# lianqi1008/Control-GIC

Measured on AMD Instinct MI355X. Metric: encode+decode MPixels/s at fixed granularity ratio; bpp match vs reference, higher is better.
Workload: dtype f32; 1 GPU; batch 64 of 256x256 per GPU per step, codebook 1024x4, ratio (0.1,0.8,0.1), hot path only (entropy maps + router + VQ + Huffman/mask coder, encode+decode); conv encoder/decoder out of scope, latent synthetic; inputs=8 distinct resident batches in rotation (416 MiB > 256 MiB Infinity Cache)

## Files before the change

control-gic_amd/csrc/cgic_decode.hip:

```cpp
#include "cgic_coder_dev.h"

#include <atomic>

namespace cgic {

constexpr int kWinBytes = 8192;
constexpr int kWinWords = kWinBytes / 4 + 4;

struct WaveDecoder {
    const TableDev &t;
    const uint32_t *lut;
    uint32_t *win;
    const uint8_t *in;
    int nbytes;
    int wb;

    __device__ __forceinline__ void fill(int first_byte)
    {
        const int lane = lane_id();
        wb = first_byte & ~3;
        const uintptr_t g = reinterpret_cast<uintptr_t>(in) + (uintptr_t)wb;
        const uint32_t *ga = reinterpret_cast<const uint32_t *>(g & ~(uintptr_t)3);
        wsh = (int)(g & 3);
        const int limit = (nbytes - wb + wsh + 3) / 4 + 2;
// ... 592 lines not shown
            decode_segmented<false>(a.tab, lut, win + wave * kSegWinWords, seg, in, nb, s_pad, 0, wave < nw ? nw : 0, wave, cap, put,
                                    &s_count, ft);
        else
            decode_segmented<true>(a.tab, lut, win + wave * kSegWinWords, seg, in, nb, s_pad, 0, wave < nw ? nw : 0, wave, cap, put,
                                   &s_count, ft);
        __syncthreads();
        if (tid == 0) *dc = s_count > cap ? -3 : s_count;
        return;
    }
    PartSync ps{a.bf + (b * 3 + s) * kDecPartsMax * kWave, a.tick + (b * 3 + s) * kTicketStride, s_entry};
    int nbits = s_pad == 0 ? 0 : (nb - 1) * 8 - s_pad;
    nbits = nbits < 0 ? 0 : nbits;
    const int nchunks = (nbits + kWave - 1) / kWave, per_part = (nchunks + nparts - 1) / nparts;
    if (per_part <= kFastChunks) {
        decode_segmented<true>(a.tab, lut, win + wave * kSegWinWords, seg, in, nb, s_pad, 0, kDecWaves, wave, cap, put, &s_count, ft,
                               part, nparts, 0, 0, nullptr, &ps);
    } else {
        decode_segmented<false>(a.tab, lut, win + wave * kSegWinWords, seg, in, nb, s_pad, 0, kDecWaves, wave, 0,
                                [](int, int) {}, &s_count, (FastTables *)nullptr, part, nparts, 0, 0, s_fn);
        __syncthreads();
        if (wave == 0) part_exchange(part, nparts, s_fn[tid], ps);
        if (tid == 0) s_count = 0;
        __syncthreads();
        decode_segmented<true>(a.tab, lut, win + wave * kSegWinWords, seg, in, nb, s_pad, 0, kDecWaves, wave, cap, put, &s_count, ft,
                               part, nparts, s_entry[0], s_entry[1]);
    }
    __syncthreads();
    if (tid == 0 && part == nparts - 1) *dc = s_count > cap ? -3 : s_count;
}

__global__ __launch_bounds__(kDecThreads) void decode_split_kernel(DecodeArgs a)
{
    decode_split_body(a, own_blk());
}

__global__ __launch_bounds__(kDecThreads) void decode_split_grouped_kernel(Grouped<DecodeArgs> g)
{
    Blk blk;
    decode_split_body(g.a[group_locate(g, &blk)], blk);
}

struct MergeArgs {
    const uint8_t *in;
    int64_t slot;
    const int32_t *nbytes;
    int64_t h, w;
    int mode;
    const uint16_t *dsym;
    const int32_t *dcount;
    int64_t *ind_out;
    int32_t *mc_out, *mm_out, *mf_out;
    const float *codebook;
    int K;
    float *zq;
    const float *codebook2;
    float *zq2;
    int32_t *status;
    int stage_sym, stage_cb;
    int64_t band_syms;
};

__device__ __forceinline__ void wait_decoded(unsigned int *done, unsigned int need, unsigned int total)
{
    if (threadIdx.x == 0) {
        while (__hip_atomic_load(done, __ATOMIC_RELAXED, __HIP_MEMORY_SCOPE_AGENT) < need) __builtin_amdgcn_s_sleep(8);
        const unsigned int old = __hip_atomic_fetch_add(done, 1u, __ATOMIC_RELAXED, __HIP_MEMORY_SCOPE_AGENT);
        if (old + 1u == total) __hip_atomic_store(done, 0u, __ATOMIC_RELAXED, __HIP_MEMORY_SCOPE_AGENT);
        __builtin_amdgcn_fence(__ATOMIC_ACQUIRE, "agent");
    }
    __syncthreads();
}

typedef unsigned int cgic_u32x4 __attribute__((ext_vector_type(4)));
typedef unsigned int cgic_u32x2 __attribute__((ext_vector_type(2)));
__device__ __forceinline__ void nt_store16(void *p, const void *v)
{
    __builtin_nontemporal_store(*reinterpret_cast<const cgic_u32x4 *>(v), reinterpret_cast<cgic_u32x4 *>(p));
}
__device__ __forceinline__ void nt_store8(void *p, const void *v)
{
    __builtin_nontemporal_store(*reinterpret_cast<const cgic_u32x2 *>(v), reinterpret_cast<cgic_u32x2 *>(p));
}

template <int NT, bool WAIT = false>
__device__ __forceinline__ void merge_body(const MergeArgs &a, const Blk blk, unsigned int *done = nullptr, unsigned int need = 0,
                                           unsigned int total = 0)
{
    extern __shared__ __attribute__((aligned(16))) uint32_t sm[];
    __shared__ uint32_t scan_smem[NT / kWave + 1];
    __shared__ int s_status;
    __shared__ int s_hdr[8];
    const int tid = threadIdx.x;
    const int band = blk.x;
    const int64_t b = blk.y;
    const int64_t h = a.h, w = a.w, h2 = h >> 1, w2 = w >> 1, h4 = h >> 2, w4 = w >> 2;
    const int64_t n_c = h4 * w4, n_m = h2 * w2, n_f = h * w;
    const int64_t wc = (n_c + 31) >> 5, wm = (n_m + 31) >> 5;
    const int64_t nsym = n_c + n_m + n_f;
    float4 *cbk = reinterpret_cast<float4 *>(sm);
    uint16_t *lsym = reinterpret_cast<uint16_t *>(cbk + (a.stage_cb ? a.K : 0));
    uint32_t *rawc = reinterpret_cast<uint32_t *>(lsym) + (a.stage_sym ? (nsym + 1) / 2 : 0);
    uint32_t *rawm = rawc + wc + 2;
    uint32_t *mcb = rawm + wm + 2;
    uint32_t *mmb = mcb + wc;
    uint32_t *pcb = mmb + wm;
    uint32_t *pmb = pcb + wc;
    const int mode = a.mode;
    const int64_t nbands = blk.nx;
    const int64_t rows_per = ((h4 + nbands - 1) / nbands) * 4;
    const int64_t r0 = band * rows_per, r1 = r0 + rows_per < h ? r0 + rows_per : h;
    if (r0 >= h) return;
    CGIC_STAMP(10);
    const bool send_mc = mode == 0 || mode == 2 || mode == 3;
    const bool send_mm = mode == 0 || mode == 1;
    const uint8_t *in_mc = a.in + (b * CGIC_NUM_STREAMS + 3) * a.slot;
    const uint8_t *in_mm = a.in + (b * CGIC_NUM_STREAMS + 4) * a.slot;

    if (tid == 0) s_status = 0;
    if (tid < 2) s_hdr[tid] = a.nbytes[b * CGIC_NUM_STREAMS + 3 + tid];
    else if (!WAIT && tid < 5) s_hdr[tid] = a.dcount[b * 3 + (tid - 2)];
    if (send_mc) for (int64_t i = tid; i < wc + 2; i += NT) rawc[i] = reinterpret_cast<const uint32_t *>(in_mc)[i];
    if (send_mm) for (int64_t i = tid; i < wm + 2; i += NT) rawm[i] = reinterpret_cast<const uint32_t *>(in_mm)[i];
    const uint16_t *gsym = a.dsym + b * nsym;
    if (!WAIT && a.stage_sym) {
        const uint32_t *g32 = reinterpret_cast<const uint32_t *>(gsym);
        uint32_t *l32 = reinterpret_cast<uint32_t *>(lsym);
        for (int64_t i = tid; i < (nsym + 1) / 2; i += NT) l32[i] = g32[i];
    }
    if (a.stage_cb && a.zq)
        for (int i = tid; i < a.K; i += NT) cbk[i] = reinterpret_cast<const float4 *>(a.codebook)[i];
    __syncthreads();
    CGIC_STAMP(11);

    if (tid == 0) {
        if (send_mc && (s_hdr[0] != 2 + (n_c >> 3) || (int)(rawc[0] & 0xFF) != 8 - (int)(n_c & 7))) s_status = CGIC_ERR_INVALID;
        if (send_mm && (s_hdr[1] != 2 + (n_m >> 3) || (int)(rawm[0] & 0xFF) != 8 - (int)(n_m & 7))) s_status = CGIC_ERR_INVALID;
    }
    __syncthreads();
    if (s_status) {
        if (WAIT) wait_decoded(done, need, total);
        if (tid == 0 && a.status) atomicMin(&a.status[b], s_status);
        return;
    }
    auto stream_word = [](const uint32_t *raw, int64_t wi, int64_t nbits) -> uint32_t {
        const uint64_t two = (uint64_t)raw[wi] | ((uint64_t)raw[wi + 1] << 32);
        const uint32_t pay = (uint32_t)(two >> 8);
        uint32_t v = __builtin_bswap32(__brev(pay));
        const int64_t rem = nbits - wi * 32;
        if (rem < 32) v &= rem <= 0 ? 0u : ((1u << rem) - 1u);
        return v;
    };
    uint32_t cnt_c, cnt_m;
    __shared__ uint32_t s_cnt[2];
    const bool derived_mm = mode == 3 || mode == 5;
    if (wc <= kWave && wm <= kWave && !derived_mm) {
        const int lane = lane_id(), wave = tid >> 6;
        if (wave < 2) {
            const bool co = wave == 0;
            const int64_t nw_ = co ? wc : wm, nb_ = co ? n_c : n_m;
            uint32_t v = 0;
            if (lane < nw_) {
                if (co ? send_mc : send_mm) v = stream_word(co ? rawc : rawm, lane, nb_);
                else if (co && mode == 4) {
                    v = 0xFFFFFFFFu;
                    const int64_t rem = nb_ - (int64_t)lane * 32;
                    if (rem < 32) v &= (1u << rem) - 1u;
                }
            }
            const uint32_t c = (uint32_t)__popc(v);
            const uint32_t inc = wave_inclusive_scan(c);
            if (lane < nw_) {
                (co ? mcb : mmb)[lane] = v;
                (co ? pcb : pmb)[lane] = inc - c;
            }
            if (lane == kWave - 1) s_cnt[wave] = inc;
        }
        __syncthreads();
        cnt_c = s_cnt[0];
        cnt_m = s_cnt[1];
    } else {
        for (int64_t i = tid; i < wc; i += NT) {
            uint32_t v = 0;
            if (send_mc) v = stream_word(rawc, i, n_c);
            else if (mode == 4) {
                v = 0xFFFFFFFFu;
                const int64_t rem = n_c - i * 32;
                if (rem < 32) v &= (1u << rem) - 1u;
            }
            mcb[i] = v;
        }
        __syncthreads();
        for (int64_t i = tid; i < wm; i += NT) {
            uint32_t v = 0;
            if (send_mm) v = stream_word(rawm, i, n_m);
            else if (mode == 3 || mode == 5) {
                for (int k = 0; k < 32; ++k) {
                    const int64_t j = i * 32 + k;
                    if (j >= n_m) break;
                    bool bit = true;
                    if (mode == 3) {
                        const int64_t y = j / w2, x = j - y * w2, c = (y >> 1) * w4 + (x >> 1);
                        bit = !((mcb[c >> 5] >> (c & 31)) & 1u);
                    }
                    v |= (uint32_t)bit << k;
                }
            }
            mmb[i] = v;
        }
        __syncthreads();
        if (wc <= NT && wm <= NT) {
            __shared__ unsigned long long scan64[NT / kWave + 1];
            const unsigned long long c = ((unsigned long long)(tid < wc ? __popc(mcb[tid]) : 0) << 32) | (unsigned long long)(tid < wm ? __popc(mmb[tid]) : 0);
            unsigned long long tot;
            const unsigned long long ex = block_exclusive_scan(c, scan64, &tot);
            if (tid < wc) pcb[tid] = (uint32_t)(ex >> 32);
            if (tid < wm) pmb[tid] = (uint32_t)ex;
            cnt_c = (uint32_t)(tot >> 32);
            cnt_m = (uint32_t)tot;
            __syncthreads();
        } else {
        uint32_t carry = 0, total;
        for (int64_t base = 0; base < wc; base += NT) {
            const int64_t i = base + tid;
            const uint32_t c = i < wc ? (uint32_t)__popc(mcb[i]) : 0u;
            const uint32_t ex = block_exclusive_scan(c, scan_smem, &total);
            if (i < wc) pcb[i] = carry + ex;
            carry += total;
        }
        cnt_c = carry;
        carry = 0;
        for (int64_t base = 0; base < wm; base += NT) {
            const int64_t i = base + tid;
            const uint32_t c = i < wm ? (uint32_t)__popc(mmb[i]) : 0u;
            const uint32_t ex = block_exclusive_scan(c, scan_smem, &total);
            if (i < wm) pmb[i] = carry + ex;
            carry += total;
        }
        cnt_m = carry;
        __syncthreads();
        }
    }
    CGIC_STAMP(12);

    auto fine_flag = [&](int64_t y, int64_t x, bool *pbc, bool *pbm) -> bool {
        const int64_t j2 = (y >> 1) * w2 + (x >> 1), j4 = (y >> 2) * w4 + (x >> 2);
        const bool bc = (mcb[j4 >> 5] >> (j4 & 31)) & 1u;
        const bool bm = (mmb[j2 >> 5] >> (j2 & 31)) & 1u;
        *pbc = bc; *pbm = bm;
        switch (mode) {
        case 0: return (1 - (int)bm - (int)bc) == 1;
        case 1: return !bm;
        case 2: return !bc;
        case 6: return true;
        default: return false;
        }
    };
    uint32_t fbase = 0;
    {
        uint32_t mine = 0;
        const int wvm = tid >> 6, lnm = tid & 63;
        for (int y2 = wvm; y2 < (int)(r0 >> 1); y2 += NT / 64)
            for (int x2 = lnm; x2 < (int)w2; x2 += 64) {
                bool bc, bm;
                mine += fine_flag(2 * y2, 2 * x2, &bc, &bm) ? 4u : 0u;
            }
        (void)block_exclusive_scan(mine, scan_smem, &fbase);
    }
    CGIC_STAMP(13);
    if (WAIT) {
        wait_decoded(done, need, total);
        if (tid >= 2 && tid < 5) s_hdr[tid] = a.dcount[b * 3 + (tid - 2)];
        if (a.stage_sym) {
            const uint32_t *g32 = reinterpret_cast<const uint32_t *>(gsym);
            uint32_t *l32 = reinterpret_cast<uint32_t *>(lsym);
            for (int64_t i = tid; i < (nsym + 1) / 2; i += NT) l32[i] = g32[i];
        }
        __syncthreads();
    }

    const uint16_t *ds_c = a.stage_sym ? lsym : gsym, *ds_m = ds_c + n_c, *ds_f = ds_m + n_m;
    const int64_t dc_c = s_hdr[2], dc_m = s_hdr[3], dc_f = s_hdr[4];
    uint16_t *bsym = reinterpret_cast<uint16_t *>(pmb + wm);
    int64_t off_c = 0, off_m = 0, off_f = 0;
    if (!a.stage_sym && a.band_syms > 0) {
        auto rank_of = [&](const uint32_t *bits, const uint32_t *pre, int64_t j, int64_t nbits, uint32_t total) -> int64_t {
            if (j >= nbits) return (int64_t)total;
            return (int64_t)pre[j >> 5] + __popc(bits[j >> 5] & ((1u << (j & 31)) - 1u));
        };
        const int64_t c0 = rank_of(mcb, pcb, (r0 >> 2) * w4, n_c, cnt_c), c1 = rank_of(mcb, pcb, (r1 >> 2) * w4, n_c, cnt_c);
        const int64_t m0 = rank_of(mmb, pmb, (r0 >> 1) * w2, n_m, cnt_m), m1 = rank_of(mmb, pmb, (r1 >> 1) * w2, n_m, cnt_m);
        const int64_t f0 = fbase, f1 = f0 + (r1 - r0) * w;
        const int64_t nc = c1 - c0, nm = m1 - m0, nf = (f1 < n_f ? f1 : n_f) - f0;
        if (nc >= 0 && nm >= 0 && nf >= 0 && nc + nm + nf + 3 <= a.band_syms) {
            for (int64_t i = tid; i < nc; i += NT) bsym[i] = ds_c[c0 + i];
            for (int64_t i = tid; i < nm; i += NT) bsym[nc + i] = ds_m[m0 + i];
            for (int64_t i = tid; i < nf; i += NT) bsym[nc + nm + i] = ds_f[f0 + i];
            __syncthreads();
            off_c = c0; off_m = m0 - nc; off_f = f0 - nc - nm;
            ds_c = bsym; ds_m = bsym; ds_f = bsym;
        }
    }
    const bool has_c = mode == 0 || mode == 2 || mode == 3 || mode == 4;
    const bool has_m = mode == 0 || mode == 1 || mode == 3 || mode == 5;
    const bool has_f = mode == 0 || mode == 1 || mode == 2 || mode == 6;
    int st = 0;
    if (dc_c == -3 || dc_m == -3 || dc_f == -3) st = CGIC_ERR_INVALID;
    if (has_c && dc_c >= 0 && dc_c != cnt_c) st = CGIC_ERR_INVALID;
    if (has_m && dc_m >= 0 && dc_m != cnt_m) st = CGIC_ERR_INVALID;
    const bool use_c = has_c && dc_c >= 0, use_m = has_m && dc_m >= 0, use_f = has_f && dc_f >= 0;

    int64_t *ind_out = a.ind_out ? a.ind_out + b * n_f : nullptr;
    float *zq = a.zq ? a.zq + b * 4 * n_f : nullptr;
    float *zq2 = a.zq2 ? a.zq2 + b * 4 * n_f : nullptr;
    uint32_t fcarry = fbase;
    int bad_index = 0;
    const int w4i = (int)w4;
    for (int64_t qbase = r0 * w4; qbase < r1 * w4; qbase += NT) {
        const int64_t q = qbase + tid;
        const bool live = q < r1 * w4;
        int64_t v[4] = {0, 0, 0, 0};
        bool bfa = false, bfb = false;
        int y = 0, xq = 0;
        if (live) {
            y = (int)q / w4i; xq = (int)q - y * w4i;
            const int64_t j4 = (int64_t)(y >> 2) * w4 + xq, j2 = (int64_t)(y >> 1) * w2 + 2 * xq;
            bool bc, bma, bmb, dummy;
            bfa = fine_flag(y, 4 * xq, &bc, &bma);
            bfb = fine_flag(y, 4 * xq + 2, &dummy, &bmb);
            int64_t vc = 0, va = 0, vb = 0;
            if (bc && use_c) vc = ds_c[(int64_t)pcb[j4 >> 5] + __popc(mcb[j4 >> 5] & ((1u << (j4 & 31)) - 1u)) - off_c];
            if (use_m) {
                const uint32_t word = mmb[j2 >> 5], below = word & ((1u << (j2 & 31)) - 1u);
                const int64_t rk = (int64_t)pmb[j2 >> 5] + __popc(below) - off_m;
                if (bma) va = ds_m[rk];
                if (bmb) vb = ds_m[rk + (bma ? 1 : 0)];
            }
            v[0] = v[1] = vc + va;
            v[2] = v[3] = vc + vb;
            const int64_t i = (int64_t)y * w + 4 * xq;
            if (a.mc_out && (y & 3) == 0) a.mc_out[b * n_c + j4] = bc;
            if (a.mm_out && (y & 1) == 0) { const int2 t2 = make_int2(bma, bmb); nt_store8(a.mm_out + b * n_m + j2, &t2); }
            if (a.mf_out) { const int4 t4 = make_int4(bfa, bfa, bfb, bfb); nt_store16(a.mf_out + b * n_f + i, &t4); }
        }
        uint32_t ftotal;
        uint32_t frank = block_exclusive_scan((bfa ? 2u : 0u) + (bfb ? 2u : 0u), scan_smem, &ftotal) + fcarry;
        if (live) {
            if (bfa) {
                if (use_f) {
                    if ((int64_t)frank < dc_f) v[0] += ds_f[(int64_t)frank - off_f];
                    if ((int64_t)frank + 1 < dc_f) v[1] += ds_f[(int64_t)frank + 1 - off_f];
                }
                frank += 2;
            }
            if (bfb && use_f) {
                if ((int64_t)frank < dc_f) v[2] += ds_f[(int64_t)frank - off_f];
                if ((int64_t)frank + 1 < dc_f) v[3] += ds_f[(int64_t)frank + 1 - off_f];
            }
            const int64_t i = (int64_t)y * w + 4 * xq;
            if (ind_out) {
                nt_store16(ind_out + i, &v[0]);
                nt_store16(ind_out + i + 2, &v[2]);
            }
            if (zq || zq2) {
#pragma unroll
                for (int k = 0; k < 4; ++k)
                    if (v[k] < 0 || v[k] >= a.K) { bad_index = 1; v[k] = 0; }
            }
            if (zq) {
                float4 e[4];
#pragma unroll
                for (int k = 0; k < 4; ++k) e[k] = a.stage_cb ? cbk[v[k]] : reinterpret_cast<const float4 *>(a.codebook)[v[k]];
                const float4 o0 = make_float4(e[0].x, e[1].x, e[2].x, e[3].x), o1 = make_float4(e[0].y, e[1].y, e[2].y, e[3].y);
                const float4 o2 = make_float4(e[0].z, e[1].z, e[2].z, e[3].z), o3 = make_float4(e[0].w, e[1].w, e[2].w, e[3].w);
                nt_store16(zq + i, &o0);
                nt_store16(zq + n_f + i, &o1);
                nt_store16(zq + 2 * n_f + i, &o2);
                nt_store16(zq + 3 * n_f + i, &o3);
            }
            if (zq2) {
                float4 e[4];
#pragma unroll
                for (int k = 0; k < 4; ++k) e[k] = reinterpret_cast<const float4 *>(a.codebook2)[v[k]];
                *reinterpret_cast<float4 *>(zq2 + i) = make_float4(e[0].x, e[1].x, e[2].x, e[3].x);
                *reinterpret_cast<float4 *>(zq2 + n_f + i) = make_float4(e[0].y, e[1].y, e[2].y, e[3].y);
                *reinterpret_cast<float4 *>(zq2 + 2 * n_f + i) = make_float4(e[0].z, e[1].z, e[2].z, e[3].z);
                *reinterpret_cast<float4 *>(zq2 + 3 * n_f + i) = make_float4(e[0].w, e[1].w, e[2].w, e[3].w);
            }
        }
        fcarry += ftotal;
    }
    CGIC_STAMP(14);
    if (r1 == h && has_f && (dc_f >= 0 ? dc_f != (int64_t)fcarry : fcarry != 0)) st = CGIC_ERR_INVALID;
    if (bad_index) s_status = CGIC_ERR_INVALID;
    __syncthreads();
    if (tid == 0 && a.status && (st || s_status)) atomicMin(&a.status[b], st ? st : s_status);
}

template <int NT>
__global__ __launch_bounds__(NT) void merge_kernel(MergeArgs a)
{
    merge_body<NT>(a, own_blk());
}

__global__ __launch_bounds__(kMergeThreads) void merge_grouped_kernel(Grouped<MergeArgs> g)
{
    Blk blk;
    merge_body<kMergeThreads>(g.a[group_locate(g, &blk)], blk);
}

struct DecodeMergeArgs {
    DecodeArgs c;
    MergeArgs m;
    unsigned int *done;
    unsigned int ndec, nbands, active_bands, B;
};
__device__ __forceinline__ void decode_merge_body(const DecodeMergeArgs &p, const unsigned int id)
{
    const unsigned int ndec_all = p.ndec * p.B;
    if (id < ndec_all) {
        const unsigned int b = id / p.ndec;
        decode_split_body(p.c, Blk{id - b * p.ndec, b, 0u, p.ndec, p.B});
        __syncthreads();
        if (threadIdx.x == 0) {
            __builtin_amdgcn_fence(__ATOMIC_RELEASE, "agent");
            __hip_atomic_fetch_add(p.done + (size_t)b * kTicketStride, 1u, __ATOMIC_RELAXED, __HIP_MEMORY_SCOPE_AGENT);
        }
        return;
    }
    const unsigned int r = id - ndec_all, b = r / p.nbands;
    merge_body<kDecThreads, true>(p.m, Blk{r - b * p.nbands, b, 0u, p.nbands, p.B}, p.done + (size_t)b * kTicketStride, p.ndec,
                                  p.ndec + p.active_bands);
}
__global__ __launch_bounds__(kDecThreads) void decode_merge_kernel(DecodeMergeArgs p)
{
    decode_merge_body(p, blockIdx.x);
}
__global__ __launch_bounds__(kDecThreads) void decode_merge_grouped_kernel(Grouped<DecodeMergeArgs> g)
{
    Blk blk;
    const DecodeMergeArgs &p = g.a[group_locate(g, &blk)];
    decode_merge_body(p, blk.x);
}

__global__ void gather_kernel(const int64_t *__restrict__ ind, int64_t B, int64_t hw,
                              const float *__restrict__ cb, int K, float *__restrict__ out,
                              int32_t *__restrict__ status)
{
    const int64_t n = B * hw;
    for (int64_t i = (int64_t)blockIdx.x * blockDim.x + threadIdx.x; i < n; i += (int64_t)gridDim.x * blockDim.x) {
        int64_t v = ind[i];
        const int64_t b = i / hw, p = i - b * hw;
        if (v < 0 || v >= K) { if (status) status[b] = CGIC_ERR_INVALID; v = 0; }
        const float4 e = reinterpret_cast<const float4 *>(cb)[v];
        float *o = out + b * 4 * hw + p;
        o[0] = e.x; o[hw] = e.y; o[2 * hw] = e.z; o[3 * hw] = e.w;
    }
}

}

using namespace cgic;

static size_t decoder_lds_bytes(bool fast_tables)
{
    const size_t seg = sizeof(uint32_t) * (kDecLutMax + kDecWaves * kSegWinWords) + sizeof(SegShared) + sizeof(int32_t) * 2 * kLdsTrieNodes
                       + (fast_tables ? sizeof(FastTables) : 0);
    const size_t one_wave = sizeof(uint32_t) * (kDecLutMax + kWinWords);
    return seg > one_wave ? seg : one_wave;
}

extern "C" int cgic_decode_stream(const cgic_table *t, const uint8_t *in, int64_t nbytes, int64_t *syms,
                                  int64_t cap, int64_t *count, cgic_stream_t stream)
{
    CGIC_NOT_IN_GROUP("cgic_decode_stream");
    CGIC_REQUIRE(t && count && (in || nbytes == 0) && (syms || cap == 0), CGIC_ERR_INVALID, "decode_stream: NULL argument");
    CGIC_REQUIRE(nbytes >= 0 && cap >= 0 && nbytes < ((int64_t)1 << 28), CGIC_ERR_INVALID, "decode_stream: size out of range");
    DecodeOneArgs a;
    int rc = table_device_view(t, &a.tab);
    if (rc) return rc;
    a.in = in; a.nbytes = nbytes; a.syms = syms; a.cap = cap; a.count = count;
    const size_t lds = decoder_lds_bytes(false);
    rc = ensure_dynamic_lds((const void *)decode_stream_kernel, lds);
    if (rc) return rc;
    hipLaunchKernelGGL(decode_stream_kernel, dim3(1), dim3(kDecThreads), lds, (hipStream_t)stream, a);
    return launch_check("decode_stream_kernel");
}

static std::atomic<int> g_decode_mode{CGIC_DECODE_AUTO};
static std::atomic<unsigned int *> g_decode_stats{nullptr};
extern "C" int cgic_decode_stats(unsigned int *device_counters)
{
    CGIC_REQUIRE(((uintptr_t)device_counters & 3u) == 0, CGIC_ERR_INVALID, "decode_stats: the counters must be 4-byte aligned");
    g_decode_stats.store(device_counters, std::memory_order_relaxed);
    return CGIC_OK;
}
extern "C" int cgic_set_decode_mode(int mode)
{
    CGIC_REQUIRE(mode == CGIC_DECODE_AUTO || mode == CGIC_DECODE_LATENCY || mode == CGIC_DECODE_THROUGHPUT, CGIC_ERR_INVALID,
                 "set_decode_mode: mode %d", mode);
    return g_decode_mode.exchange(mode);
}

extern "C" size_t cgic_decompress_workspace_bytes(int64_t B, int64_t h, int64_t w)
{
    if (B <= 0 || h <= 0 || w <= 0) return 0;
    const size_t per = (size_t)((h / 4) * (w / 4) + (h / 2) * (w / 2) + h * w);
    return align16((size_t)B * per * sizeof(uint16_t)) + align16((size_t)B * 3 * sizeof(int32_t))
           + align16((size_t)B * 3 * kDecPartsMax * kWave * sizeof(uint32_t));
}

extern "C" int cgic_decompress_streams(const cgic_table *t, const uint8_t *in, int64_t slot, const int32_t *nbytes,
                                       int64_t B, int64_t h, int64_t w, int mode, int64_t *ind_out,
                                       int32_t *mask_c_out, int32_t *mask_m_out, int32_t *mask_f_out,
                                       const float *codebook, int K, int e_dim, float *z_q, const float *codebook2,
                                       float *z_q2, int32_t *status,
                                       void *workspace, int decoder, cgic_stream_t stream)
{
    int rc = check_grid(B, h, w, mode);
    if (rc) return rc;
    CGIC_REQUIRE(t && in && nbytes && workspace, CGIC_ERR_INVALID, "decompress_streams: NULL argument");
    CGIC_REQUIRE(decoder == CGIC_DECODE_AUTO || decoder == CGIC_DECODE_LATENCY || decoder == CGIC_DECODE_THROUGHPUT, CGIC_ERR_INVALID,
                 "decompress_streams: decoder %d", decoder);
    const int dec_mode = decoder != CGIC_DECODE_AUTO ? decoder : g_decode_mode.load();
    CGIC_REQUIRE(slot % 16 == 0 && slot >= 16 && slot < ((int64_t)1 << 28), CGIC_ERR_INVALID,
                 "decompress_streams: slot must be a multiple of 16 below 2^28");
    CGIC_REQUIRE(!z_q || (codebook && e_dim == 4 && K > 0), CGIC_ERR_UNSUPPORTED,
                 "decompress_streams: fused gather needs a [K,4] codebook");
    CGIC_REQUIRE(!z_q2 || (codebook2 && e_dim == 4 && K > 0), CGIC_ERR_UNSUPPORTED,
                 "decompress_streams: the second gather needs a [K,4] table");
    CGIC_REQUIRE(cgic_table_num_symbols(t) <= 65536, CGIC_ERR_UNSUPPORTED, "table too large");
    CGIC_REQUIRE(((reinterpret_cast<uintptr_t>(ind_out) | reinterpret_cast<uintptr_t>(z_q) | reinterpret_cast<uintptr_t>(z_q2) |
                   reinterpret_cast<uintptr_t>(mask_f_out)) & 15) == 0 && (reinterpret_cast<uintptr_t>(mask_m_out) & 7) == 0,
                 CGIC_ERR_INVALID, "decompress_streams: outputs must be 16-byte aligned");
    if (B == 0) return CGIC_OK;
    hipStream_t s = (hipStream_t)stream;
    DecodeArgs d;
    rc = table_device_view(t, &d.tab);
    if (rc) return rc;

    DecodeShape shape;
    shape.B = B; shape.h = h; shape.w = w; shape.slot = slot; shape.K = K; shape.has_zq = z_q != nullptr;
    shape.max_len = d.tab.max_len; shape.lut_bits = d.tab.lut_bits; shape.dec_mode = dec_mode;
    rc = device_cu_count(&shape.cus);
    if (rc) return rc;
// ... 116 lines not shown
```

control-gic_amd/csrc/cgic_decode_ss.hip:

```cpp
#include "cgic_coder_dev.h"

namespace cgic {

constexpr int kSsEnd = 0xFF;

struct SsLayout {
    int nbits[3];
    int c[4];
    int off[3];
};
__device__ __forceinline__ int sel3(int s, int v0, int v1, int v2) { return s == 0 ? v0 : (s == 1 ? v1 : v2); }

__device__ __forceinline__ uint32_t ss_bits(uint32_t d0, uint32_t d1, uint32_t d2, int pos)
{
    const uint32_t hi = pos < 32 ? d0 : d1, lo = pos < 32 ? d1 : d2;
    const uint32_t r = __builtin_amdgcn_alignbit(hi, lo, 32u - ((uint32_t)pos & 31u));
    return (pos & 31) ? r : hi;
}

template <bool WRITE, typename Put>
__device__ __forceinline__ int ss_walk(const TableDev &t, const uint32_t *lut, const uint8_t *stage, const SsLayout &L, int g,
                                       int entry, int *count, Put put)
{
    const int s = (g >= L.c[1]) + (g >= L.c[2]);
    const int ch = g - sel3(s, L.c[0], L.c[1], L.c[2]);
    const int rem = sel3(s, L.nbits[0], L.nbits[1], L.nbits[2]) - 64 * ch;
    *count = 0;
    if (entry == kSsEnd) return kSsEnd;
    const uint32_t *q = reinterpret_cast<const uint32_t *>(stage + sel3(s, L.off[0], L.off[1], L.off[2]) + 8 * ch);
    const uint32_t r0 = __builtin_bswap32(q[0]), r1 = __builtin_bswap32(q[1]), r2 = __builtin_bswap32(q[2]),
                   r3 = __builtin_bswap32(q[3]), r4 = __builtin_bswap32(q[4]);
    const uint32_t d0 = __builtin_amdgcn_alignbit(r0, r1, 24), d1 = __builtin_amdgcn_alignbit(r1, r2, 24),
                   d2 = __builtin_amdgcn_alignbit(r2, r3, 24), d3 = __builtin_amdgcn_alignbit(r3, r4, 24);
    const int LB = t.lut_bits;
    int pos = entry, n = 0;
    if (t.max_len <= LB) {
        const uint32_t a0 = pos < 32 ? d0 : d1, a1 = pos < 32 ? d1 : d2, a2 = pos < 32 ? d2 : d3, a3 = pos < 32 ? d3 : 0u;
        const uint32_t sft = 32u - ((uint32_t)pos & 31u);
        const bool al = ((uint32_t)pos & 31u) == 0u;
        uint32_t w0 = al ? a0 : __builtin_amdgcn_alignbit(a0, a1, sft), w1 = al ? a1 : __builtin_amdgcn_alignbit(a1, a2, sft),
                 w2 = al ? a2 : __builtin_amdgcn_alignbit(a2, a3, sft);
        const int remc = rem < 128 ? rem : 128, lim = rem < 64 ? rem : 64;
        const uint32_t ish = 30u - (uint32_t)LB;
        const uint32_t imask = ((1u << LB) - 1u) << 2;
        const char *lutb = reinterpret_cast<const char *>(lut);
        auto step = [&]() {
            const bool go = pos < lim;
            const uint32_t e = *reinterpret_cast<const uint32_t *>(lutb + ((w0 >> ish) & imask));
            const int len = (int)(e & 0xFF);
            const int np = pos + len;
            const bool ok = go && np <= remc;
            if (WRITE) { if (ok) put(s, n, (int)(e >> 8)); }
            const uint32_t r = 32u - (uint32_t)len;
            w0 = __builtin_amdgcn_alignbit(w0, w1, r);
            w1 = __builtin_amdgcn_alignbit(w1, w2, r);
            w2 <<= (len & 31);
            pos = go ? np : pos;
            n += ok ? 1 : 0;
        };
        while (__builtin_amdgcn_ballot_w64(pos < lim) != 0) {
            step();
            step();
        }
        *count = n;
        return (pos < 64 || pos > remc) ? kSsEnd : pos - 64;
    }
    while (pos < 64) {
        if (pos >= rem) { *count = n; return kSsEnd; }
        const uint32_t bits = ss_bits(d0, d1, d2, pos);
        const uint32_t e = lut[bits >> (32 - LB)];
        int len = (int)(e & 0xFF), sym = (int)(e >> 8);
        if (len == 0) {
            if (sym == 0xFFFFFF) { *count = n; return kSsEnd; }
            const unsigned long long w0 = ((unsigned long long)d0 << 32) | d1, w1 = ((unsigned long long)d2 << 32) | d3;
            const unsigned long long win = pos ? (w0 << pos) | (w1 >> (64 - pos)) : w0;
            int node = sym, k = LB;
            sym = -1;
            while (pos + k < rem && k < 64) {
                const int c = t.child[2 * node + (int)((win >> (63 - k)) & 1ull)];
                ++k;
                if (c == INT32_MIN) break;
                if (c < 0) { sym = ~c; break; }
                node = c;
            }
            if (sym < 0) { *count = n; return kSsEnd; }
            len = k;
        }
        if (pos + len > rem) { *count = n; return kSsEnd; }
        if (WRITE) put(s, n, sym);
        pos += len;
        ++n;
    }
    *count = n;
    return pos - 64;
}


constexpr int kSsMaxSweeps = 32;
constexpr int kMeEntries = 15;
constexpr uint32_t kMeEnd = 15;

struct MeFn { uint32_t r[4]; };

__device__ __forceinline__ MeFn me_identity() { return MeFn{{0x03020100u, 0x07060504u, 0x0B0A0908u, 0x0F0E0D0Cu}}; }
__device__ __forceinline__ MeFn me_const0() { return MeFn{{0u, 0u, 0u, 0u}}; }
__device__ __forceinline__ MeFn me_compose(const MeFn &prev, const MeFn &cur)
{
    MeFn o;
#pragma unroll
    for (int k = 0; k < 4; ++k) {
        const uint32_t sel = prev.r[k];
        const uint32_t s7 = sel & 0x07070707u;
        const uint32_t lo = __builtin_amdgcn_perm(cur.r[1], cur.r[0], s7);
        const uint32_t hi = __builtin_amdgcn_perm(cur.r[3], cur.r[2], s7);
        const uint32_t m = ((sel >> 3) & 0x01010101u) * 0xFFu;
        o.r[k] = (hi & m) | (lo & ~m);
    }
    return o;
}
__device__ __forceinline__ uint32_t me_apply(const MeFn &f, uint32_t e)
{
    const uint32_t w = e < 8 ? (e < 4 ? f.r[0] : f.r[1]) : (e < 12 ? f.r[2] : f.r[3]);
    return (w >> (8 * (e & 3))) & 0xFFu;
}
__device__ __forceinline__ MeFn me_shfl_up(const MeFn &f, int d)
{
    MeFn o;
#pragma unroll
    for (int k = 0; k < 4; ++k) o.r[k] = (uint32_t)__shfl_up((int)f.r[k], d, kWave);
    return o;
}
__device__ __forceinline__ MeFn me_wave_scan(MeFn f)
{
    const int lane = lane_id();
#pragma unroll
    for (int d = 1; d < kWave; d <<= 1) {
        const MeFn p = me_shfl_up(f, d);
        const MeFn c = me_compose(p, f);
        if (lane >= d) f = c;
    }
    return f;
}

__device__ __forceinline__ MeFn me_walk_all(const TableDev &t, const uint32_t *lut, const uint8_t *stage, const SsLayout &L, int g,
                                            unsigned long long *cnt_lo, unsigned long long *cnt_hi)
{
    const int s = (g >= L.c[1]) + (g >= L.c[2]);
    const int ch = g - sel3(s, L.c[0], L.c[1], L.c[2]);
    const int rem = sel3(s, L.nbits[0], L.nbits[1], L.nbits[2]) - 64 * ch;
    const uint32_t *q = reinterpret_cast<const uint32_t *>(stage + sel3(s, L.off[0], L.off[1], L.off[2]) + 8 * ch);
    const uint32_t r0 = __builtin_bswap32(q[0]), r1 = __builtin_bswap32(q[1]), r2 = __builtin_bswap32(q[2]), r3 = __builtin_bswap32(q[3]);
    const uint32_t d0 = __builtin_amdgcn_alignbit(r0, r1, 24), d1 = __builtin_amdgcn_alignbit(r1, r2, 24), d2 = __builtin_amdgcn_alignbit(r2, r3, 24);
    const int LB = t.lut_bits;
    const int remc = rem < 128 ? rem : 128, lim = rem < 64 ? rem : 64;
    const uint32_t ish = 30u - (uint32_t)LB, imask = ((1u << LB) - 1u) << 2;
    const char *lutb = reinterpret_cast<const char *>(lut);
    const int E = t.max_len < kMeEntries ? t.max_len : kMeEntries;
    int pos[kMeEntries], n[kMeEntries];
#pragma unroll
    for (int e = 0; e < kMeEntries; ++e) { pos[e] = e < E ? e : 1 << 20; n[e] = 0; }
    for (;;) {
        bool any = false;
#pragma unroll
        for (int e = 0; e < kMeEntries; ++e) any |= pos[e] < lim;
        if (__builtin_amdgcn_ballot_w64(any) == 0) break;
#pragma unroll
        for (int e = 0; e < kMeEntries; ++e) {
            const int p = pos[e];
            const bool go = p < lim;
            const uint32_t bits = ss_bits(d0, d1, d2, p & 63);
            const uint32_t ent = *reinterpret_cast<const uint32_t *>(lutb + ((bits >> ish) & imask));
            const int np = p + (int)(ent & 0xFF);
            const bool ok = go && np <= remc;
            pos[e] = go ? np : p;
            n[e] += ok ? 1 : 0;
        }
    }
    MeFn f;
    unsigned long long lo = 0, hi = 0;
#pragma unroll
    for (int k = 0; k < 4; ++k) f.r[k] = 0;
#pragma unroll
    for (int e = 0; e < kMeEntries; ++e) {
        const int p = pos[e];
        const uint32_t x = (e >= E || p < 64 || p > remc) ? kMeEnd : (uint32_t)(p - 64);
        f.r[e >> 2] |= x << (8 * (e & 3));
        if (e < 8) lo |= (unsigned long long)(uint32_t)n[e] << (8 * e);
        else hi |= (unsigned long long)(uint32_t)n[e] << (8 * (e - 8));
    }
    f.r[3] |= kMeEnd << 24;
    *cnt_lo = lo; *cnt_hi = hi;
    return f;
}

__device__ __forceinline__ void decode_image_body(const DecodeArgs &a, const int stage_cap, const int chunk_cap, const Blk blk)
{
    extern __shared__ __attribute__((aligned(16))) uint32_t sm[];
    __shared__ int s_scan[kDecWaves + 1];
    __shared__ int s_base[4];
    __shared__ MeFn s_fn[kDecWaves];
    uint32_t *lut = sm;
    uint8_t *stage = reinterpret_cast<uint8_t *>(lut + (1 << a.tab.lut_bits));
    uint8_t *ent = stage + stage_cap, *ext = ent + chunk_cap, *cnt = ext + chunk_cap;
    const int tid = threadIdx.x, T = blockDim.x, lane = lane_id(), wave = tid >> 6, nw = T >> 6;
    const int64_t b = blk.x;
    CGIC_STAMP3(0);
    const uint8_t *in0 = a.in + (b * CGIC_NUM_STREAMS) * a.slot;
    int nb[3];
#pragma unroll
    for (int s = 0; s < 3; ++s) nb[s] = (a.stream_mask >> s & 1) ? a.nbytes[b * CGIC_NUM_STREAMS + s] : -2;
    const int pad[3] = {in0[0], in0[a.slot], in0[2 * a.slot]};
    {
        const uint4 *gl = reinterpret_cast<const uint4 *>(a.tab.lut);
        uint4 *dl = reinterpret_cast<uint4 *>(lut);
        const int n4 = (1 << a.tab.lut_bits) >> 2;
        const bool mark = a.tab.max_len <= a.tab.lut_bits;
        auto fix = [mark](uint32_t e) { return mark && (e & 0xFFu) == 0u ? e | 0xFFu : e; };
        if (n4 == 0 && tid < (1 << a.tab.lut_bits)) lut[tid] = fix(a.tab.lut[tid]);
        for (int base = 0; base < n4; base += 8 * T) {
            uint4 v[8];
#pragma unroll
            for (int k = 0; k < 8; ++k) {
                const int i = base + k * T + tid;
                v[k] = i < n4 ? gl[i] : uint4{0u, 0u, 0u, 0u};
            }
#pragma unroll
            for (int k = 0; k < 8; ++k) {
                const int i = base + k * T + tid;
                if (i < n4) dl[i] = uint4{fix(v[k].x), fix(v[k].y), fix(v[k].z), fix(v[k].w)};
            }
        }
    }
    const int64_t n_c = (a.h >> 2) * (a.w >> 2), n_m = (a.h >> 1) * (a.w >> 1), n_f = a.h * a.w;
    const int cap[3] = {(int)n_c, (int)n_m, (int)n_f};
    SsLayout L;
    int stage_used = 0;
    bool fits = true;
    L.c[0] = 0;
#pragma unroll
    for (int s = 0; s < 3; ++s) {
        if (nb[s] > a.slot) nb[s] = (int)a.slot;
        int bits = nb[s] <= 0 || pad[s] == 0 ? 0 : (nb[s] - 1) * 8 - pad[s];
        bits = bits < 0 ? 0 : bits;
        L.nbits[s] = bits;
        L.c[s + 1] = L.c[s] + ((bits + 63) >> 6);
        L.off[s] = stage_used;
        stage_used += bits ? (((bits + 7) >> 3) + 1 + 24 + 15) & ~15 : 0;
    }
    const int C = L.c[3];
    if (stage_used > stage_cap || C > chunk_cap) fits = false;
    if (tid == 0) {
        if (a.status) a.status[b] = 0;
#pragma unroll
        for (int s = 0; s < 3; ++s) {
            if (nb[s] <= 0) a.dcount[b * 3 + s] = nb[s] == 0 ? -1 : -2;
            else if (!fits) a.dcount[b * 3 + s] = -3;
        }
    }
    if (!fits) return;
    CGIC_STAMP3(1);
#pragma unroll
    for (int s = 0; s < 3; ++s) {
        if (!L.nbits[s]) continue;
        const int words = ((((L.nbits[s] + 7) >> 3) + 1 + 24 + 15) & ~15) >> 4;
        const uint4 *g = reinterpret_cast<const uint4 *>(in0 + s * a.slot);
        uint4 *d = reinterpret_cast<uint4 *>(stage + L.off[s]);
        const int lim = (int)(a.slot >> 4);
        for (int i = tid; i < words; i += T) d[i] = i < lim ? g[i] : uint4{0u, 0u, 0u, 0u};
    }
    __syncthreads();
    CGIC_STAMP3(2);
    const int R = (C + T - 1) / T;
    const int g0 = tid * R < C ? tid * R : C, g1 = g0 + R < C ? g0 + R : C;
    auto is_first = [&](int g) { return g == L.c[0] || g == L.c[1] || g == L.c[2]; };
    auto nop = [](int, int, int) {};
    int dbg_sweeps = 0;
    const bool all_entries = a.tab.max_len <= a.tab.lut_bits && a.tab.max_len <= kMeEntries;
    bool stuck = false;
    {
        int prev = 0;
        for (int g = g0; g < g1; ++g) {
            int e = prev;
            if (is_first(g)) e = 0;
            else if (g == g0) {
                const int sg = (g >= L.c[1]) + (g >= L.c[2]);
                const int chg = g - sel3(sg, L.c[0], L.c[1], L.c[2]);
                const int m = (64 * chg) % a.tab.len_gcd;
                e = m ? a.tab.len_gcd - m : 0;
            }
            int n;
            prev = ss_walk<false>(a.tab, lut, stage, L, g, e, &n, nop);
            ent[g] = (uint8_t)e; ext[g] = (uint8_t)prev; cnt[g] = (uint8_t)n;
        }
    }
    __syncthreads();
    CGIC_STAMP3(3);
    for (;;) {
        ++dbg_sweeps;
        int changed = 0;
        for (int g = g0; g < g1; ++g) {
            const int e = is_first(g) ? 0 : ext[g - 1];
            if (e != ent[g]) {
                int n;
                const int x = ss_walk<false>(a.tab, lut, stage, L, g, e, &n, nop);
                ent[g] = (uint8_t)e; ext[g] = (uint8_t)x; cnt[g] = (uint8_t)n;
                changed = 1;
            }
        }
        if (!__syncthreads_or(changed)) break;
        if (all_entries && dbg_sweeps >= kSsMaxSweeps) { stuck = true; break; }
    }
    if (stuck) {
        MeFn mine = me_identity();
        unsigned long long c_lo = 0, c_hi = 0;
        for (int g = g0; g < g1; ++g) {
            MeFn f = me_walk_all(a.tab, lut, stage, L, g, &c_lo, &c_hi);
            if (is_first(g + 1)) f = me_const0();
            mine = me_compose(mine, f);
        }
        const MeFn incl = me_wave_scan(mine);
        if (lane == kWave - 1) s_fn[wave] = incl;
        __syncthreads();
        MeFn before = me_identity();
        for (int w2 = 0; w2 < wave; ++w2) before = me_compose(before, s_fn[w2]);
        MeFn prev = me_shfl_up(incl, 1);
        if (lane == 0) prev = me_identity();
        uint32_t e = me_apply(prev, me_apply(before, 0u));
        if (g0 < g1 && is_first(g0)) e = 0;
        if (R == 1) {
            if (g0 < g1) {
                const unsigned long long cw = e < 8 ? c_lo : c_hi;
                ent[g0] = (uint8_t)(e == kMeEnd ? kSsEnd : (int)e);
                cnt[g0] = e == kMeEnd ? (uint8_t)0 : (uint8_t)((cw >> (8 * (e & 7))) & 0xFFull);
            }
        } else {
            int en = e == kMeEnd ? kSsEnd : (int)e;
            for (int g = g0; g < g1; ++g) {
                if (is_first(g)) en = 0;
                int n;
                const int x = ss_walk<false>(a.tab, lut, stage, L, g, en, &n, nop);
                ent[g] = (uint8_t)en; cnt[g] = (uint8_t)n;
                en = x;
            }
        }
        dbg_sweeps += 1;
        __syncthreads();
    }
    CGIC_STAMP3(4);
    if (a.stats && tid == 0) {
        atomicAdd(&a.stats[0], (unsigned int)dbg_sweeps);
        atomicAdd(&a.stats[1], 1u);
        atomicMax(&a.stats[2], (unsigned int)dbg_sweeps);
    }
#ifdef CGIC_PHASE_CLOCKS
    if (blk.x == 0 && tid == 0) g_phase_clk[9] = dbg_sweeps;
#endif
    int mine = 0;
    for (int g = g0; g < g1; ++g) mine += cnt[g];
    int inc = wave_inclusive_scan(mine);
    if (lane == kWave - 1) s_scan[wave] = inc;
    __syncthreads();
    if (wave == 0) {
        const int v = lane < nw ? s_scan[lane] : 0;
        const int vi = wave_inclusive_scan(v);
        if (lane < nw) s_scan[lane] = vi - v;
        if (lane == nw - 1) s_scan[kDecWaves] = vi;
    }
    __syncthreads();
    int run = s_scan[wave] + inc - mine;
    const int total = s_scan[kDecWaves];
    {
        int r = run;
        for (int g = g0; g < g1; ++g) {
            if (g == L.c[1]) s_base[1] = r;
            if (g == L.c[2]) s_base[2] = r;
            r += cnt[g];
        }
        if (tid == 0) {
            s_base[0] = 0; s_base[3] = total;
            if (L.c[2] == C) s_base[2] = total;
            if (L.c[1] == C) s_base[1] = total;
        }
    }
    __syncthreads();
    CGIC_STAMP3(5);
    uint16_t *dst = a.dsym + b * (n_c + n_m + n_f);
    for (int g = g0; g < g1; ++g) {
        const int s = (g >= L.c[1]) + (g >= L.c[2]);
        const int at = run - s_base[s];
        const int cap_s = sel3(s, cap[0], cap[1], cap[2]);
        uint16_t *dst_s = dst + sel3(s, 0, (int)n_c, (int)(n_c + n_m)) + at;
        int n;
        ss_walk<true>(a.tab, lut, stage, L, g, (int)ent[g], &n,
                      [&](int, int k, int sym) { if (at + k < cap_s) dst_s[k] = (uint16_t)sym; });
        run += n;
    }
    CGIC_STAMP3(6);
    if (tid < 3 && sel3(tid, nb[0], nb[1], nb[2]) > 0) {
        const int n = s_base[tid + 1] - s_base[tid];
        a.dcount[b * 3 + tid] = n > sel3(tid, cap[0], cap[1], cap[2]) ? -3 : n;
    }
}

__global__ __launch_bounds__(kDecThreads) void decode_image_kernel(DecodeArgs a, int stage_cap, int chunk_cap)
{
    decode_image_body(a, stage_cap, chunk_cap, own_blk());
}

__global__ __launch_bounds__(kDecThreads) void decode_image_grouped_kernel(Grouped<DecodeImageArgs> g)
{
    Blk blk;
    const DecodeImageArgs &p = g.a[group_locate(g, &blk)];
    decode_image_body(p.a, p.stage_cap, p.chunk_cap, blk);
}

}

using namespace cgic;
static GroupedRegistrar reg_decode_image(KID_DECODE_IMAGE, [](const GroupRec *const *recs, int n, hipStream_t s) {
    return launch_grouped(decode_image_grouped_kernel, "decode_image_grouped_kernel", recs[0]->block, LDS_ALWAYS, recs, n, s); });
```

Measured before the change: 127,700 MPixels/s.

## Replace per-row fine-mask block scans with precomputed prefix bitmaps; cache SS windows in registers

When both coarse and medium masks fit in one wave's worth of words, a third wave builds a packed fine-flag bitmap by expanding the coarse mask bits and combining them with the medium mask. It then prefix-scans that bitmap, so each thread can compute its fine-symbol rank directly with popcounts. This replaces the per-row block-wide exclusive scan and the initial counting loop, removing repeated barriers. In the self-synchronising Huffman decoder, the R==1 path keeps its bitstream window, entry and count in registers instead of reloading from the stage buffer and shared arrays on each sweep. This adds some per-thread register pressure and extra work for the third wave.

```diff
diff --git a/control-gic_amd/csrc/cgic_decode.hip b/control-gic_amd/csrc/cgic_decode.hip
--- a/control-gic_amd/csrc/cgic_decode.hip
+++ b/control-gic_amd/csrc/cgic_decode.hip
@@ -768,9 +768,49 @@
     };
     uint32_t cnt_c, cnt_m;
     __shared__ uint32_t s_cnt[2];
+    __shared__ uint32_t ffb[kWave + 1], pfb[kWave + 1];
     const bool derived_mm = mode == 3 || mode == 5;
-    if (wc <= kWave && wm <= kWave && !derived_mm) {
+    const bool small_masks = wc <= kWave && wm <= kWave && !derived_mm;
+    if (small_masks) {
         const int lane = lane_id(), wave = tid >> 6;
+        if (wave == 2) {
+            uint32_t f = 0;
+            if (lane < wm) {
+                const int j0 = lane * 32, nv = (int)n_m - j0 < 32 ? (int)n_m - j0 : 32;
+                const uint32_t mmw = send_mm ? stream_word(rawm, lane, n_m) : 0u;
+                uint32_t up = 0;
+                if (mode == 0 || mode == 2) {
+                    const int w2i = (int)w2, w4i_ = (int)w4;
+                    int y2 = j0 / w2i, x2 = j0 - y2 * w2i;
+                    for (int p = 0; p < nv; ++y2, x2 = 0) {
+                        const int n = w2i - x2 < nv - p ? w2i - x2 : nv - p;
+                        const int c0 = (y2 >> 1) * w4i_ + (x2 >> 1), k = c0 >> 5;
+                        const uint64_t two = (uint64_t)stream_word(rawc, k, n_c) | (k + 1 < wc ? (uint64_t)stream_word(rawc, k + 1, n_c) << 32 : 0ull);
+                        uint32_t sp = (uint32_t)(two >> (c0 & 31)) & 0xFFFFu;
+                        sp = (sp | (sp << 8)) & 0x00FF00FFu;
+                        sp = (sp | (sp << 4)) & 0x0F0F0F0Fu;
+                        sp = (sp | (sp << 2)) & 0x33333333u;
+                        sp = (sp | (sp << 1)) & 0x55555555u;
+                        sp |= sp << 1;
+                        if (n < 32) sp &= (1u << n) - 1u;
+                        up |= sp << p;
+                        p += n;
+                    }
+                }
+                switch (mode) {
+                case 0: f = ~(mmw | up); break;
+                case 1: f = ~mmw; break;
+                case 2: f = ~up; break;
+                case 6: f = 0xFFFFFFFFu; break;
+                default: break;
+                }
+                if (nv < 32) f &= (1u << nv) - 1u;
+            }
+            const uint32_t c = (uint32_t)__popc(f);
+            const uint32_t inc = wave_inclusive_scan(c);
+            if (lane < wm) { ffb[lane] = f; pfb[lane + 1] = inc; }
+            if (lane == 0) { pfb[0] = 0u; ffb[wm] = 0u; }
+        }
         if (wave < 2) {
             const bool co = wave == 0;
             const int64_t nw_ = co ? wc : wm, nb_ = co ? n_c : n_m;
@@ -872,7 +912,12 @@
         }
     };
     uint32_t fbase = 0;
-    {
+    auto fine_cells_before = [&](int j) -> uint32_t {
+        return pfb[j >> 5] + (uint32_t)__popc(ffb[j >> 5] & ((1u << (j & 31)) - 1u));
+    };
+    if (small_masks) {
+        fbase = 4u * fine_cells_before((int)(r0 >> 1) * (int)w2);
+    } else {
         uint32_t mine = 0;
         const int wvm = tid >> 6, lnm = tid & 63;
         for (int y2 = wvm; y2 < (int)(r0 >> 1); y2 += NT / 64)
@@ -958,8 +1003,19 @@
             if (a.mm_out && (y & 1) == 0) { const int2 t2 = make_int2(bma, bmb); nt_store8(a.mm_out + b * n_m + j2, &t2); }
             if (a.mf_out) { const int4 t4 = make_int4(bfa, bfa, bfb, bfb); nt_store16(a.mf_out + b * n_f + i, &t4); }
         }
-        uint32_t ftotal;
-        uint32_t frank = block_exclusive_scan((bfa ? 2u : 0u) + (bfb ? 2u : 0u), scan_smem, &ftotal) + fcarry;
+        uint32_t frank = 0;
+        if (small_masks) {
+            if (live) {
+                const int row = (y >> 1) * (int)w2;
+                const uint32_t p0 = fine_cells_before(row), pr = fine_cells_before(row + 2 * xq);
+                frank = 2u * (p0 + pr);
+                if (y & 1) frank += 2u * (fine_cells_before(row + (int)w2) - p0);
+            }
+        } else {
+            uint32_t ftotal;
+            frank = block_exclusive_scan((bfa ? 2u : 0u) + (bfb ? 2u : 0u), scan_smem, &ftotal) + fcarry;
+            fcarry += ftotal;
+        }
         if (live) {
             if (bfa) {
                 if (use_f) {
@@ -1003,9 +1059,9 @@
                 *reinterpret_cast<float4 *>(zq2 + 3 * n_f + i) = make_float4(e[0].w, e[1].w, e[2].w, e[3].w);
             }
         }
-        fcarry += ftotal;
     }
     CGIC_STAMP(14);
+    if (small_masks) fcarry = 4u * pfb[wm];
     if (r1 == h && has_f && (dc_f >= 0 ? dc_f != (int64_t)fcarry : fcarry != 0)) st = CGIC_ERR_INVALID;
     if (bad_index) s_status = CGIC_ERR_INVALID;
     __syncthreads();
diff --git a/control-gic_amd/csrc/cgic_decode_ss.hip b/control-gic_amd/csrc/cgic_decode_ss.hip
--- a/control-gic_amd/csrc/cgic_decode_ss.hip
+++ b/control-gic_amd/csrc/cgic_decode_ss.hip
@@ -18,20 +18,56 @@
     return (pos & 31) ? r : hi;
 }
 
+struct SsWin {
+    int s, rem;
+    uint32_t d0, d1, d2, d3;
+};
+__device__ __forceinline__ void ss_locate(const SsLayout &L, int g, SsWin *W, int *ch)
+{
+    W->s = (g >= L.c[1]) + (g >= L.c[2]);
+    *ch = g - sel3(W->s, L.c[0], L.c[1], L.c[2]);
+    W->rem = sel3(W->s, L.nbits[0], L.nbits[1], L.nbits[2]) - 64 * *ch;
+}
+__device__ __forceinline__ void ss_load(const uint8_t *stage, const SsLayout &L, int ch, SsWin *W)
+{
+    const uint32_t *q = reinterpret_cast<const uint32_t *>(stage + sel3(W->s, L.off[0], L.off[1], L.off[2]) + 8 * ch);
+    const uint32_t r0 = __builtin_bswap32(q[0]), r1 = __builtin_bswap32(q[1]), r2 = __builtin_bswap32(q[2]),
+                   r3 = __builtin_bswap32(q[3]), r4 = __builtin_bswap32(q[4]);
+    W->d0 = __builtin_amdgcn_alignbit(r0, r1, 24); W->d1 = __builtin_amdgcn_alignbit(r1, r2, 24);
+    W->d2 = __builtin_amdgcn_alignbit(r2, r3, 24); W->d3 = __builtin_amdgcn_alignbit(r3, r4, 24);
+}
+__device__ __forceinline__ SsWin ss_window(const uint8_t *stage, const SsLayout &L, int g)
+{
+    SsWin W;
+    int ch;
+    ss_locate(L, g, &W, &ch);
+    ss_load(stage, L, ch, &W);
+    return W;
+}
+
+template <bool WRITE, typename Put>
+__device__ __forceinline__ int ss_walk_from(const TableDev &t, const uint32_t *lut, const SsWin &W, int entry, int *count, Put put);
+
 template <bool WRITE, typename Put>
 __device__ __forceinline__ int ss_walk(const TableDev &t, const uint32_t *lut, const uint8_t *stage, const SsLayout &L, int g,
                                        int entry, int *count, Put put)
 {
-    const int s = (g >= L.c[1]) + (g >= L.c[2]);
-    const int ch = g - sel3(s, L.c[0], L.c[1], L.c[2]);
-    const int rem = sel3(s, L.nbits[0], L.nbits[1], L.nbits[2]) - 64 * ch;
+    SsWin W;
+    int ch;
+    ss_locate(L, g, &W, &ch);
     *count = 0;
     if (entry == kSsEnd) return kSsEnd;
-    const uint32_t *q = reinterpret_cast<const uint32_t *>(stage + sel3(s, L.off[0], L.off[1], L.off[2]) + 8 * ch);
-    const uint32_t r0 = __builtin_bswap32(q[0]), r1 = __builtin_bswap32(q[1]), r2 = __builtin_bswap32(q[2]),
-                   r3 = __builtin_bswap32(q[3]), r4 = __builtin_bswap32(q[4]);
-    const uint32_t d0 = __builtin_amdgcn_alignbit(r0, r1, 24), d1 = __builtin_amdgcn_alignbit(r1, r2, 24),
-                   d2 = __builtin_amdgcn_alignbit(r2, r3, 24), d3 = __builtin_amdgcn_alignbit(r3, r4, 24);
+    ss_load(stage, L, ch, &W);
+    return ss_walk_from<WRITE>(t, lut, W, entry, count, put);
+}
+
+template <bool WRITE, typename Put>
+__device__ __forceinline__ int ss_walk_from(const TableDev &t, const uint32_t *lut, const SsWin &W, int entry, int *count, Put put)
+{
+    const int s = W.s, rem = W.rem;
+    const uint32_t d0 = W.d0, d1 = W.d1, d2 = W.d2, d3 = W.d3;
+    *count = 0;
+    if (entry == kSsEnd) return kSsEnd;
     const int LB = t.lut_bits;
     int pos = entry, n = 0;
     if (t.max_len <= LB) {
@@ -277,7 +313,22 @@
     int dbg_sweeps = 0;
     const bool all_entries = a.tab.max_len <= a.tab.lut_bits && a.tab.max_len <= kMeEntries;
     bool stuck = false;
-    {
+    const bool one = R == 1;
+    const bool own = g0 < g1;
+    SsWin W1 = {0, 0, 0u, 0u, 0u, 0u};
+    int ent1 = kSsEnd, cnt1 = 0;
+    bool first1 = false;
+    if (one) {
+        if (own) {
+            W1 = ss_window(stage, L, g0);
+            first1 = is_first(g0);
+            if (!first1) {
+                const int m = (64 * (g0 - sel3(W1.s, L.c[0], L.c[1], L.c[2]))) % a.tab.len_gcd;
+                ent1 = m ? a.tab.len_gcd - m : 0;
+            } else ent1 = 0;
+            ext[g0] = (uint8_t)ss_walk_from<false>(a.tab, lut, W1, ent1, &cnt1, nop);
+        }
+    } else {
         int prev = 0;
         for (int g = g0; g < g1; ++g) {
             int e = prev;
@@ -298,6 +349,16 @@
     for (;;) {
         ++dbg_sweeps;
         int changed = 0;
+        if (one) {
+            if (own) {
+                const int e = first1 ? 0 : ext[g0 - 1];
+                if (e != ent1) {
+                    ent1 = e;
+                    ext[g0] = (uint8_t)ss_walk_from<false>(a.tab, lut, W1, e, &cnt1, nop);
+                    changed = 1;
+                }
+            }
+        } else
         for (int g = g0; g < g1; ++g) {
             const int e = is_first(g) ? 0 : ext[g - 1];
             if (e != ent[g]) {
@@ -330,8 +391,8 @@
         if (R == 1) {
             if (g0 < g1) {
                 const unsigned long long cw = e < 8 ? c_lo : c_hi;
-                ent[g0] = (uint8_t)(e == kMeEnd ? kSsEnd : (int)e);
-                cnt[g0] = e == kMeEnd ? (uint8_t)0 : (uint8_t)((cw >> (8 * (e & 7))) & 0xFFull);
+                ent1 = e == kMeEnd ? kSsEnd : (int)e;
+                cnt1 = e == kMeEnd ? 0 : (int)((cw >> (8 * (e & 7))) & 0xFFull);
             }
         } else {
             int en = e == kMeEnd ? kSsEnd : (int)e;
@@ -355,8 +416,8 @@
 #ifdef CGIC_PHASE_CLOCKS
     if (blk.x == 0 && tid == 0) g_phase_clk[9] = dbg_sweeps;
 #endif
-    int mine = 0;
-    for (int g = g0; g < g1; ++g) mine += cnt[g];
+    int mine = one ? cnt1 : 0;
+    if (!one) for (int g = g0; g < g1; ++g) mine += cnt[g];
     int inc = wave_inclusive_scan(mine);
     if (lane == kWave - 1) s_scan[wave] = inc;
     __syncthreads();
@@ -374,7 +435,7 @@
         for (int g = g0; g < g1; ++g) {
             if (g == L.c[1]) s_base[1] = r;
             if (g == L.c[2]) s_base[2] = r;
-            r += cnt[g];
+            r += one ? cnt1 : (int)cnt[g];
         }
         if (tid == 0) {
             s_base[0] = 0; s_base[3] = total;
@@ -391,8 +452,9 @@
         const int cap_s = sel3(s, cap[0], cap[1], cap[2]);
         uint16_t *dst_s = dst + sel3(s, 0, (int)n_c, (int)(n_c + n_m)) + at;
         int n;
-        ss_walk<true>(a.tab, lut, stage, L, g, (int)ent[g], &n,
-                      [&](int, int k, int sym) { if (at + k < cap_s) dst_s[k] = (uint16_t)sym; });
+        auto store = [&](int, int k, int sym) { if (at + k < cap_s) dst_s[k] = (uint16_t)sym; };
+        if (one) ss_walk_from<true>(a.tab, lut, W1, ent1, &n, store);
+        else ss_walk<true>(a.tab, lut, stage, L, g, (int)ent[g], &n, store);
         run += n;
     }
     CGIC_STAMP3(6);
```

After: 128,900 MPixels/s (median of 5 runs). Within noise of the previous version (+0.9%).
